# mjuvela/SOC

Hardware: AMD Instinct MI355X
Metric: photon packets/sec (higher is better)
Workload: dtype f32

## Files before the change

### soc_amd/csrc/soc_brick.hip

```cpp
#include "soc_walk.h"
#include "soc_ltree.h"

#include <cstdio>
#include <algorithm>
#include <chrono>
#include <cstdlib>
#include <cstring>
#include <vector>

#include "soc_lbricks.h"

#define SOC_BRICK_T 256

#if defined(SOC_BRICK_PROF)
__device__ unsigned long long g_soc_prof[24];
#define SOC_PROF_DECL unsigned int prof_[8] = { 0, 0, 0, 0, 0, 0, 0, 0 }, dprof_[8] = { 0, 0, 0, 0, 0, 0, 0, 0 };  unsigned long long tprof_[8] = { 0, 0, 0, 0, 0, 0, 0, 0 }, tlast_ = __builtin_readcyclecounter()
#define SOC_PROF_T(i) do { const unsigned long long t_ = __builtin_readcyclecounter();  tprof_[i] += t_ - tlast_;  tlast_ = t_; } while (0)
#define SOC_PROF_ENTRY const unsigned long long tentry_ = __builtin_readcyclecounter()
#define SOC_PROF_SINCE_ENTRY(i) do { tprof_[i] += tlast_ - tentry_; } while (0)
#define SOC_PROF(i, n) do { prof_[i] += (unsigned int)(n); } while (0)
#define SOC_DPROF(i, n) do { dprof_[i] += (unsigned int)(n); } while (0)
#define SOC_PROF_FLUSH do { if ((threadIdx.x & 63) == 0) for (int i_ = 0; i_ < 8; i_++) atomicAdd(&g_soc_prof[16 + i_], (unsigned long long)dprof_[i_]); \
                            if ((threadIdx.x & 63) == 0) for (int i_ = 0; i_ < 8; i_++) atomicAdd(&g_soc_prof[i_], (unsigned long long)prof_[i_]); \
                            if ((threadIdx.x & 63) == 0) for (int i_ = 0; i_ < 8; i_++) atomicAdd(&g_soc_prof[8 + i_], tprof_[i_]); } while (0)
extern "C" __attribute__((visibility("default"))) void soc_prof_read(unsigned long long *out, int reset)
{
    (void)hipMemcpyFromSymbol(out, HIP_SYMBOL(g_soc_prof), sizeof(unsigned long long) * 24);
    if (reset) { unsigned long long z[24] = { 0 };  (void)hipMemcpyToSymbol(HIP_SYMBOL(g_soc_prof), z, sizeof(z)); }
}
#else
#define SOC_PROF_DECL
#define SOC_PROF_ENTRY
#define SOC_PROF_SINCE_ENTRY(i) do { } while (0)
#define SOC_PROF_T(i) do { } while (0)
#define SOC_PROF(i, n) do { } while (0)
#define SOC_DPROF(i, n) do { } while (0)
#define SOC_PROF_FLUSH do { } while (0)
#endif
#define SOC_BRICK_PMAX 4096
#define SOC_RANK_BITS 16
#define SOC_LBRICK_PMAX 32768

enum { SOC_BM_STEP = 0, SOC_BM_CLIMB = 1, SOC_BM_SWAP = 3, SOC_BM_IDLE = 4 };

struct __align__(16) SocPk2 { float4 A, B, C; uint4 D; };

struct SocDesc { int brick, start, count, pad; };

#if defined(SOC_BRICK_NT)
#define SOC_NT_LOAD(p)      __builtin_nontemporal_load(p)
#define SOC_NT_STORE(v, p)  __builtin_nontemporal_store((v), (p))
#else
#define SOC_NT_LOAD(p)      (*(p))
#define SOC_NT_STORE(v, p)  (*(p) = (v))
#endif
typedef float soc_f4v __attribute__((ext_vector_type(4)));
typedef uint32_t soc_u2v __attribute__((ext_vector_type(2)));
#define SOC_GLOBAL __attribute__((address_space(1)))
#define SOC_CHUNK_AT(base, slot) ((decltype(base))((SOC_GLOBAL const char *)(base) + (uint32_t)((uint32_t)(slot) << 2)))
#define SOC_TAKE(dst, src) asm volatile("v_mov_b32 %0, %1" : "=v"(dst) : "v"(src))
__device__ __forceinline__ float4 soc_ld4(const float4 *p) { const soc_f4v v = SOC_NT_LOAD((const soc_f4v *)p);  return make_float4(v.x, v.y, v.z, v.w); }
__device__ __forceinline__ void soc_st4(float4 *p, float4 a) { soc_f4v v = { a.x, a.y, a.z, a.w };  SOC_NT_STORE(v, (soc_f4v *)p); }

struct SocBrickArgs {
    int LB, NBX, NBY, NBZ, NB;
    int NBQ;
    int T, P, KCAP, FTH;
    int CTH;
    int TAIL;
    int PARK;
    SocPk2 *pk;
    const uint32_t *idq;
    uint32_t *idq_next;
    uint32_t *keyq;
    uint32_t *posq;
    int *hist;
    int *off;
    const SocDesc *desc;
    const int *ndesc;
    SocDesc *desc_next;
    int *ndesc_next;
    int *total;
    int ev_brick;
    int HS;
    long long opt_stride;
    int target, nl;
    const uint32_t *first;
    int *admit;
    int CAP;
    const float2 *DS;
    float sib_thr;
    const int *bcell;
    const int *bbase;
    int LT;
    int EQ;
    int slow_every;
    const SocLBrick *lbr;
    const float *btree;
    const int *rbrick;
    int kexp;
    int int_only;
    int ali;
    int roi_on;
    SocPk2 *park;
    SocSca sca;
    const float2 *kopt;
    long long kopt_stride;
};

#include "soc_octbricks.h"
#define SOC_LVL_SHIFT 16
#define SOC_LCH_SHIFT 20

__device__ __forceinline__ void soc_qh_init(int *sH, int HS, int NQ)
{
    if (HS == 0) { for (int i = threadIdx.x; i < NQ; i += blockDim.x) sH[i] = 0; }
    else         { for (int i = threadIdx.x; i < HS; i += blockDim.x) { sH[i] = -1;  sH[HS + i] = 0; } }
}
__device__ __forceinline__ int soc_qh_find(int *sH, int HS, int key)
{
    uint32_t h = (((uint32_t)key * 0x9E3779B1u) >> 12) & (uint32_t)(HS - 1);
    for (int t = 0; t < 32; t++) {
        const int old = atomicCAS(&sH[h], -1, key);
        if (old == -1 || old == key) return (int)h;
        h = (h + 1) & (uint32_t)(HS - 1);
    }
    return -1;
}
#define SOC_POS_FINAL 0x80000000u
__device__ __forceinline__ uint32_t soc_qh_rank(int *sH, int HS, int key, int *ghist)
{
    if (HS == 0) return ((uint32_t)key << SOC_RANK_BITS) | (uint32_t)atomicAdd(&sH[key], 1);
    const int h = soc_qh_find(sH, HS, key);
    if (h >= 0) return ((uint32_t)h << SOC_RANK_BITS) | (uint32_t)atomicAdd(&sH[HS + h], 1);
    return SOC_POS_FINAL | (uint32_t)atomicAdd(&ghist[key], 1);
}
__device__ __forceinline__ void soc_qh_bases(int *sH, int HS, int NQ, int *ghist)
{
    if (HS == 0) {
        for (int i = threadIdx.x; i < NQ; i += blockDim.x) { const int c = sH[i];  if (c) sH[i] = atomicAdd(&ghist[i], c); }
    } else {
        for (int i = threadIdx.x; i < HS; i += blockDim.x) { const int k = sH[i], c = sH[HS + i];  if (k >= 0 && c) sH[HS + i] = atomicAdd(&ghist[k], c); }
    }
}
__device__ __forceinline__ uint32_t soc_qh_place(const int *sH, int HS, uint32_t pack)
{
    if (pack & SOC_POS_FINAL) return pack & ~SOC_POS_FINAL;
    return (uint32_t)sH[(HS ? HS : 0) + (pack >> SOC_RANK_BITS)] + (pack & ((1u << SOC_RANK_BITS) - 1u));
}


__device__ __forceinline__ void soc_cell_brick(const SocBrickArgs &A, float px, float py, float pz, int &brick, int &lid)
{
    const int ix = (int)soc_floorf(px), iy = (int)soc_floorf(py), iz = (int)soc_floorf(pz);
    const int M = (1 << A.LB) - 1;
    brick = ((iz >> A.LB) * A.NBY + (iy >> A.LB)) * A.NBX + (ix >> A.LB);
    lid   = ((iz & M) << (2 * A.LB)) | ((iy & M) << A.LB) | (ix & M);
}

struct SocBrickLane {
    float px, py, pz, ux, uy, uz;
    float photons, free_path, tau, dens;
    int   level, ind, scat;
    soc_rng_t rng;

    __device__ __forceinline__ void begin_conditioned(const SocSim &S)
    {
        scat = 0;
        tau  = 0.0f;
        free_path = soc_draw_free_path(S, &rng, photons);
    }
    __device__ __forceinline__ void begin(const SocSim &S)
    {
        if (soc_fabsf(ux) < SOC_DEPS) ux = SOC_DEPS;
        if (soc_fabsf(uy) < SOC_DEPS) uy = SOC_DEPS;
        if (soc_fabsf(uz) < SOC_DEPS) uz = SOC_DEPS;
        soc_normalize(ux, uy, uz);
        scat = 0;
        tau  = 0.0f;
        free_path = soc_draw_free_path(S, &rng, photons);
    }
};


__global__ void soc_brick2_init(const SocSimPack *Kp, SocBrickArgs A, uint32_t count, uint32_t *idq0, SocDesc *desc0, int *ndesc0, int *hist)
{
    const SocSimPack &K = *Kp;
    const uint32_t t = blockIdx.x * blockDim.x + threadIdx.x;
    SocPk2 *pk = A.pk;
    if (t < count) {
        int l = 0, hi = K.n;
        while (hi - l > 1) { const int m = (l + hi) >> 1;  if (t >= K.first[m]) l = m; else hi = m; }
        const soc_rng_t r = soc_seed_stream(K.S[l].seed_mul, K.S[l].seed_tab, K.S[l].gid0 + (t - K.first[l]));
        SocPk2 p;
        p.A = make_float4(0.0f, 0.0f, 0.0f, 0.0f);
        p.B = p.A;
        p.C = make_float4(0.0f, 0.0f, __int_as_float(l << SOC_LCH_SHIFT), __int_as_float(-1));
        const uint32_t cell0 = (K.S[l].SOURCE == SOC_SOURCE_CL) ? (uint32_t)((int)(K.S[l].gid0 + (t - K.first[l])) - K.S[l].GLOBAL) : 0u;
        p.D = make_uint4(r.x, r.c, 0u, cell0);
        pk[t] = p;
        idq0[t] = t;
        if (A.park) { p.C = p.A;  p.D = make_uint4(0u, 0u, 0u, 0u);  A.park[t] = p; }
    }
    const uint32_t active = min(count, (uint32_t)A.target);
    uint32_t dbase = 0;
    for (int l = 0; l < K.n; l++) {
        const uint32_t hi = min(K.first[l + 1], active);
        const uint32_t cnt = (hi > K.first[l]) ? (hi - K.first[l]) : 0u;
        const uint32_t nd = (cnt + A.P - 1) / A.P;
        if (t >= dbase && t < dbase + nd) {
            const uint32_t k = t - dbase;
            SocDesc d;
            d.brick = A.NBQ + A.EQ * l;
// ... 176 lines not shown
                    }
                }
            }
            SOC_PROF_T(2);
            if (finish) {
                if (!CL && (level == level0) && (ind == ind0)) {
                    px += SOC_PEPS * ux;  py += SOC_PEPS * uy;  pz += SOC_PEPS * uz;
                }
                nvisit++;
                if (ind < 0) {
                    mode = SOC_BM_SWAP;  key = A.NBQ + A.EQ * (lsh >> SOC_LCH_SHIFT);
                } else {
                    const int nb = (int)(sl >> SOC_SLOT_BITS);
                    lid = (int)(sl & SOC_SLOT_MASK);
                    if (nb != mybrick || nvisit >= A.KCAP) { mode = SOC_BM_SWAP;  key = qbase + nb; }
                }
            }
        } else
        if (mode == SOC_BM_STEP) {
            const int   oind = ind, lid0 = lid;
            const float p0x = px, p0y = py, p0z = pz, d0 = dens;
            if (ABU) { float2 o = S.OPT[(lsh >> SOC_LCH_SHIFT) * A.opt_stride + oind];  kabs = o.x;  ksca = o.y; }
            float fx, fy, fz;
            if (__ballot(__builtin_fminf(px, __builtin_fminf(py, pz)) < 0.0f) == 0ull) {
                fx = __builtin_amdgcn_fractf(px);  fy = __builtin_amdgcn_fractf(py);  fz = __builtin_amdgcn_fractf(pz);
            } else {
                fx = soc_fmod1f(px);  fy = soc_fmod1f(py);  fz = soc_fmod1f(pz);
            }
            const float ax = soc_div_by_rcp(((ux > 0.0f) ? (1.0f + SOC_PEPS) : -SOC_PEPS) - fx, ux, rux);
            const float ay = soc_div_by_rcp(((uy > 0.0f) ? (1.0f + SOC_PEPS) : -SOC_PEPS) - fy, uy, ruy);
            const float az = soc_div_by_rcp(((uz > 0.0f) ? (1.0f + SOC_PEPS) : -SOC_PEPS) - fz, uz, ruz);
            float ds = __builtin_fminf(ax, __builtin_fminf(ay, az));
            px += ds * ux;
            py += ds * uy;
            pz += ds * uz;
            ds = soc_scale_down(ds, 0);
            const bool inside = (px > 0.0f) & (px < fNX) & (py > 0.0f) & (py < fNY) & (pz > 0.0f) & (pz < fNZ);
            const int ix = inside ? (int)px : 0;
            const int iy = inside ? (int)py : 0;
            const int iz = inside ? (int)pz : 0;
            const int nind = iz * NX * NY + iy * NX + ix;
            const int nb   = ((iz >> LB) * A.NBY + (iy >> LB)) * A.NBX + (ix >> LB);
            const int nlid = ((iz & M) << (2 * LB)) | ((iy & M) << LB) | (ix & M);
            const bool stay = inside & (nb == mybrick);
            const float ndens = G.DENS[nind];
            const float tauA = ds * d0 * kabs;
            const float dtau = ds * d0 * ksca;
            if (free_path < (tau + dtau)) {
                px = p0x;  py = p0y;  pz = p0z;
                mode = SOC_BM_SWAP;  key = A.NBQ + A.EQ * (lsh >> SOC_LCH_SHIFT) + 1;
            } else {
                const float e = (__ballot(!(tauA < 0.34f)) == 0ull) ? soc_expf_small(-tauA) : soc_expf(-tauA);
                const float delta = (tauA > SOC_TAULIM) ? (photons * (1.0f - e)) : (photons * tauA * (1.0f - 0.5f * tauA));
                atomicAdd(&sT[lid0], delta * tw);
                if (WINT) atomicAdd(&sI[lid0], delta);
                n_tally++;
                photons *= e;
                tau += dtau;
                ind = inside ? nind : -1;
                dens = ndens;
                lid = nlid;
                const bool failed = !CL && (ind == oind);
                px += failed ? (SOC_PEPS * ux) : 0.0f;
                py += failed ? (SOC_PEPS * uy) : 0.0f;
                pz += failed ? (SOC_PEPS * uz) : 0.0f;
                nvisit++;
                if (!inside)                          { mode = SOC_BM_SWAP;  key = A.NBQ + A.EQ * (lsh >> SOC_LCH_SHIFT); }
                else if (!stay || nvisit >= A.KCAP)   { mode = SOC_BM_SWAP;  key = qbase + nb; }
            }
        }
    }

    SOC_PROF_FLUSH;
    atomicAdd(&sCtl[1], (int)n_tally);
    __syncthreads();
    if (OCT) {
        const int *cells = A.bcell + A.bbase[mybrick];
        for (int i = threadIdx.x; i < nslot; i += nthr) {
            const float v = sT[i];
            const float vi = WINT ? sI[i] : 0.0f;
            if (v != 0.0f || vi != 0.0f) {
                const int cell = cells[i];
                soc_tally(S.TABS, cell, v);
                if (WINT) soc_tally(K.S[K.gfirst[qbase / A.NB]].INT, cell, vi);
            }
        }
    } else {
        const int B = 1 << A.LB;
        const int bx = mybrick % A.NBX, by = (mybrick / A.NBX) % A.NBY, bz = mybrick / (A.NBX * A.NBY);
        for (int i = threadIdx.x; i < BV; i += nthr) {
            const float v = sT[i];
            const float vi = WINT ? sI[i] : 0.0f;
            if (v != 0.0f || vi != 0.0f) {
                const int ix = bx * B + (i & M), iy = by * B + ((i >> A.LB) & M), iz = bz * B + (i >> (2 * A.LB));
                const int cell = iz * NX * NY + iy * NX + ix;
                soc_tally(S.TABS, cell, v);
                if (WINT) soc_tally(K.S[K.gfirst[qbase / A.NB]].INT, cell, vi);
            }
        }
    }
    soc_qh_bases(sH, A.HS, NQ, A.hist);
    __syncthreads();
    for (int j = threadIdx.x; j < D.count; j += nthr) A.posq[D.start + j] = soc_qh_place(sH, A.HS, sPos[j]);
    if (threadIdx.x == 0 && S.stats) atomicAdd(S.stats + 0, (unsigned long long)(unsigned int)sCtl[1]);
}

#define SOC_LT_ARRIVE 0x80000000u
#define SOC_LQ_SHIFT 24
enum { SOC_OC_STAY = 0, SOC_OC_OWN = 1, SOC_OC_LEAVE = 2, SOC_OC_EXIT = 3, SOC_OC_SLOW = 4, SOC_OC_LOST = 5, SOC_OC_SCAT = 6, SOC_OC_ROI = 7, SOC_OC_DONE = 8,
       SOC_OC_NONE = 9, SOC_OC_IDLE = 10 };
#define SOC_OC_EVQ 0x31020000u
#define SOC_OC_EVQ_OF(oc) ((SOC_OC_EVQ >> ((4 * (oc)) & 31)) & 15u)
static_assert(SOC_OC_EVQ_OF(SOC_OC_EXIT) == 0 && SOC_OC_EVQ_OF(SOC_OC_DONE) == 0 && SOC_OC_EVQ_OF(SOC_OC_SCAT) == 1 && SOC_OC_EVQ_OF(SOC_OC_SLOW) == 2
              && SOC_OC_EVQ_OF(SOC_OC_ROI) == 3 && SOC_OC_DONE == 8 && SOC_OC_NONE == 9, "the event queue of every code that is stored, the wrap of DONE included");
static_assert(SOC_OC_LEAVE == SOC_LT_LEAVE + 1 && SOC_OC_EXIT == SOC_LT_EXIT + 1 && SOC_OC_SLOW == SOC_LT_SLOW + 1 && SOC_OC_LOST == SOC_LT_LOST + 1, "outcome codes follow soc_ltree.h");

__device__ __forceinline__ void soc_cell_coords(const SocGrid &G, const int *sOFF, int level, int ind, int &cx, int &cy, int &cz)
{
    int x = 0, y = 0, z = 0;
    for (int j = 0; j < level; j++) {
        x |= (ind & 1) << j;  y |= ((ind >> 1) & 1) << j;  z |= ((ind >> 2) & 1) << j;
        ind = G.PAR[sOFF[level - j] + ind - G.NXYZ];
    }
    cx = x | ((ind % G.NX) << level);
    cy = y | (((ind / G.NX) % G.NY) << level);
    cz = z | ((ind / (G.NX * G.NY)) << level);
}

__device__ __forceinline__ int soc_cell_index(const SocGrid &G, int level, int cx, int cy, int cz, float &dens)
{
    int ind = ((cz >> level) * G.NY + (cy >> level)) * G.NX + (cx >> level);
    dens = G.DENS[ind];
    for (int l = 1; l <= level; l++) {
        const int sh = level - l;
        ind = soc_link_index(dens) + (((cx >> sh) & 1) | (((cy >> sh) & 1) << 1) | (((cz >> sh) & 1) << 2));
        dens = G.DENS[G.OFF[l] + ind];
    }
    return ind;
}

template <int WINT, bool ALI>
__device__ __forceinline__ void soc_lbrick_tally(float *sT, float *sI, float *sV, float *sX, const int *sC, const int BV, const int st,
                                                 const float delta, const float tw, const float ux, const float uy, const float uz, const uint32_t dw)
{
    if (ALI) atomicAdd((sC[st] == (int)dw) ? &sX[st] : &sT[st], delta * tw);
    else if (WINT != 3) atomicAdd(&sT[st], delta * tw);
    if (WINT) atomicAdd(&sI[st], delta);
    if (WINT == 2) { atomicAdd(&sV[st], delta * ux);  atomicAdd(&sV[BV + st], delta * uy);  atomicAdd(&sV[2 * BV + st], delta * uz); }
}

template <int WINT, bool RAY = false, bool ALI = false, bool LIM = false, bool CART = false, bool ABU = false, bool FLT = false>
__device__ __forceinline__ void soc_lbrick_walk(const SocGrid &G, const SocSimPack &K, const SocBrickArgs &A, const int bid)
{
    if (bid >= *A.ndesc) return;
    SocDesc D = A.desc[bid];
    D.brick = __builtin_amdgcn_readfirstlane(D.brick);  D.start = __builtin_amdgcn_readfirstlane(D.start);  D.count = __builtin_amdgcn_readfirstlane(D.count);
    if (D.brick >= A.NBQ) return;
    const bool parked = __builtin_amdgcn_readfirstlane(D.pad) != 0;
    SOC_PROF_ENTRY;
    const int BV = A.CAP;
    const int nthr = (int)blockDim.x;
    SOC_GLOBAL SocPk2 *pk = (SOC_GLOBAL SocPk2 *)A.pk;

    extern __shared__ float lds[];
    float *sT   = lds;
    float *sI   = sT + ((RAY || WINT == 3) ? 0 : BV);
    float *sV   = sI + (WINT ? BV : 0);
    float *sX   = sV + ((WINT == 2) ? 3 * BV : 0);
    int   *sC   = (int *)(sX + (ALI ? BV : 0));
    float *sD   = (float *)(sC + (ALI ? BV : 0));
    const int NQ = A.NBQ + A.EQ * A.nl + 1;
    const float2 *sK = (const float2 *)(sD + BV);
    int   *sH   = (int *)(sD + BV + (ABU ? 2 * BV : 0));
    int   *sCtl = sH + (A.HS ? 2 * A.HS : ((NQ + 3) & ~3));
    float *sL   = (float *)(sCtl + 4);
    const SocSim &S = K.S[0];
    for (int l = threadIdx.x; l < K.n; l += nthr) {
        sL[4 * l] = K.S[l].ABS;  sL[4 * l + 1] = K.S[l].SCA;  sL[4 * l + 2] = K.S[l].TW;
        sL[4 * l + 3] = __int_as_float(((K.S[l].SOURCE == SOC_SOURCE_CL) ? 1 : 0) | ((LIM && K.S[l].SCAKIND == SOC_SCA_PB + 1) ? 2 : 0));
    }
    const int mybrick = (A.NBQ > A.NB) ? (D.brick % A.NB) : D.brick;
    const int qbase = D.brick - mybrick;
    SocLBrick KB = A.lbr[mybrick];
    KB.x0 = __builtin_amdgcn_readfirstlane(KB.x0);  KB.y0 = __builtin_amdgcn_readfirstlane(KB.y0);  KB.z0 = __builtin_amdgcn_readfirstlane(KB.z0);
    KB.bx = __builtin_amdgcn_readfirstlane(KB.bx);  KB.by = __builtin_amdgcn_readfirstlane(KB.by);  KB.bz = __builtin_amdgcn_readfirstlane(KB.bz);
    KB.base = __builtin_amdgcn_readfirstlane(KB.base);  KB.nslot = __builtin_amdgcn_readfirstlane(KB.nslot);
    if (!parked) {
        const float *src = A.btree + KB.base;
        for (int i = threadIdx.x; i < KB.nslot; i += nthr) {
            sD[i] = src[i];  if (!RAY && WINT != 3) sT[i] = 0.0f;  if (WINT) sI[i] = 0.0f;
            if (WINT == 2) { sV[i] = 0.0f;  sV[BV + i] = 0.0f;  sV[2 * BV + i] = 0.0f; }
            if (ALI) { sX[i] = 0.0f;  sC[i] = A.bcell[KB.base + i]; }
        }
        if (ABU) {
            const float2 *ksrc = A.kopt + (long long)(qbase / A.NB) * A.kopt_stride + KB.base;
            float2 *dst = (float2 *)(sD + BV);
            for (int i = threadIdx.x; i < KB.nslot; i += nthr) dst[i] = ksrc[i];
        }
    }
    soc_qh_init(sH, A.HS, NQ);
    if (threadIdx.x < 2) sCtl[threadIdx.x] = 0;
    if (parked) for (int j = threadIdx.x; j < D.count; j += nthr) A.keyq[D.start + j] = (uint32_t)D.brick;
    __syncthreads();

    int NX = G.NX, NY = G.NY, NZ = G.NZ, Lmax = G.LEVELS - 1, kexp = A.kexp;
    asm volatile("" : "+s"(NX), "+s"(NY), "+s"(NZ), "+s"(Lmax), "+s"(kexp));
    int rx0 = 1, rx1 = 0, ry0 = 1, ry1 = 0, rz0 = 1, rz1 = 0;
    if (!RAY && A.roi_on) {
        const SocRoi *R = S.ROI;
        rx0 = __builtin_amdgcn_readfirstlane(R->ROI[0]);  rx1 = __builtin_amdgcn_readfirstlane(R->ROI[1]);  ry0 = __builtin_amdgcn_readfirstlane(R->ROI[2]);
        ry1 = __builtin_amdgcn_readfirstlane(R->ROI[3]);  rz0 = __builtin_amdgcn_readfirstlane(R->ROI[4]);  rz1 = __builtin_amdgcn_readfirstlane(R->ROI[5]);
    }
    SOC_GLOBAL uint32_t *keyq_c = (SOC_GLOBAL uint32_t *)(A.keyq + D.start);
    const SOC_GLOBAL uint32_t *idq_c = (const SOC_GLOBAL uint32_t *)(A.idq + D.start);
    asm volatile("" : "+s"(pk), "+s"(keyq_c), "+s"(idq_c));
    float px = 0.0f, py = 0.0f, pz = 0.0f, ux = 0.0f, uy = 0.0f, uz = 0.0f;
    float photons = 0.0f, free_path = 0.0f, tau = 0.0f, dens = 0.0f;
    float rux = 1.0f, ruy = 1.0f, ruz = 1.0f;
    float gx = 0.0f, gy = 0.0f, gz = 0.0f;
    float kabs = 0.0f, ksca = 0.0f, tw = 0.0f;
    int   cx = 0, cy = 0, cz = 0, level = 0, slot = 0, obase = 0, nvisit = 0, cslot = 0, lq = 0;
    int   kl = 0;
    int   what = SOC_LTM_STEP;
    bool  nonudge = false;
    bool  dblstep = false;
    uint32_t dz = 0, dw = 0, wid = 0;
    int   oc = SOC_OC_NONE;
    bool  have = false, nhave = false;
    soc_f4v na = { 0.0f, 0.0f, 0.0f, 0.0f }, nb = na, nc = na;
    soc_u2v ndzw = { 0u, 0u };
    uint32_t nwid = 0, nnwid = 0;
    int   nslot = 0, nnslot = 0;
    bool  nnhave = false;
    unsigned int n_tally = 0;
    SOC_PROF_DECL;
    SOC_PROF_SINCE_ENTRY(3);

    while (!parked) {
        {
            SOC_PROF(0, 1);  SOC_PROF(1, __popcll(__ballot(oc == SOC_OC_STAY)));  SOC_PROF(7, __popcll(__ballot(oc == SOC_OC_IDLE)));
            if (D.count < 4 * nthr)  { SOC_DPROF(0, 1);  SOC_DPROF(1, __popcll(__ballot(oc == SOC_OC_IDLE))); }
            if (D.count < 16 * nthr) { SOC_DPROF(2, 1);  SOC_DPROF(3, __popcll(__ballot(oc == SOC_OC_IDLE))); }
            if (__ballot(nhave | nnhave) == 0ull) { SOC_DPROF(4, 1);  SOC_DPROF(5, __popcll(__ballot(oc == SOC_OC_IDLE))); }
            if (A.TAIL > 0 && D.count >= 8 * nthr && __popcll(__ballot(oc == SOC_OC_IDLE)) >= A.TAIL
                && oc == SOC_OC_STAY && what == SOC_LTM_STEP && nvisit > 0) oc = SOC_OC_OWN;
            const unsigned long long m = __ballot(oc - 1u < (unsigned)SOC_OC_NONE);
            const bool nobody_steps = (__ballot(oc == SOC_OC_STAY) == 0ull);
            if (m != 0ull && (nobody_steps || __popcll(m) >= A.FTH)) {
                SOC_PROF(4, 1);  SOC_PROF(5, __popcll(m));
                if (oc - 1u < (unsigned)SOC_OC_NONE) {
                    const int n_res = atomicAdd(&sCtl[0], 1);
                    const int  n_cz = __float_as_int(nc.w);
                    const int  n_lq = (int)(((uint32_t)n_cz >> SOC_LQ_SHIFT) & (SOC_MAXLAUNCH - 1));
                    const bool n_arrive = (ndzw.y & SOC_LT_ARRIVE) != 0u;
                    const int  n_level = (int)(ndzw.x >> 29);
                    const int  n_ix = n_arrive ? (int)soc_floorf(na.x) : __float_as_int(nc.y), n_iy = n_arrive ? (int)soc_floorf(na.y) : __float_as_int(nc.z),
                               n_iz = n_arrive ? (int)soc_floorf(na.z) : (n_cz & ((1 << SOC_LQ_SHIFT) - 1));
                    int n_s2 = SOC_MAD24(SOC_MAD24(n_iz - KB.z0, KB.by, n_iy - KB.y0), KB.bx, n_ix - KB.x0);
                    n_s2 = ((unsigned)n_s2 < (unsigned)KB.nslot) ? n_s2 : 0;
                    const soc_f4v l4 = *(const soc_f4v *)&sL[4 * n_lq];
                    const float n_rec = sD[n_s2];
                    if (have) {
                        SOC_GLOBAL SocPk2 *q = pk + wid;
                        { const soc_f4v v = { px, py, pz, photons };  SOC_NT_STORE(v, (SOC_GLOBAL soc_f4v *)&q->A); }
                        { const soc_f4v v = { tau, __int_as_float(cx), __int_as_float(cy), __int_as_float(cz | (lq << SOC_LQ_SHIFT)) };  SOC_NT_STORE(v, (SOC_GLOBAL soc_f4v *)&q->C); }
                        q->D.z = dz | ((uint32_t)level << 29);
                        q->D.w = dw | (((oc == SOC_OC_LEAVE) | (oc == SOC_OC_SLOW)) ? SOC_LT_ARRIVE : 0u);
                        if (LIM) SOC_NT_STORE(free_path, &q->B.w);
                        const int evk = A.NBQ + A.EQ * lq + (int)SOC_OC_EVQ_OF(oc);
                        const int key = (oc == SOC_OC_OWN) ? D.brick : ((oc == SOC_OC_LEAVE) ? kl : ((oc == SOC_OC_LOST) ? (NQ - 1) : evk));
                        SOC_NT_STORE((uint32_t)key, SOC_CHUNK_AT(keyq_c, cslot));
                    }
                    have = nhave;
                    wid = nwid;  cslot = nslot;
                    SOC_TAKE(px, na.x);  SOC_TAKE(py, na.y);  SOC_TAKE(pz, na.z);  SOC_TAKE(photons, na.w);
                    SOC_TAKE(ux, nb.x);  SOC_TAKE(uy, nb.y);  SOC_TAKE(uz, nb.z);  SOC_TAKE(free_path, nb.w);
                    SOC_TAKE(tau, nc.x);
                    dz = ndzw.x & 0x1fffffffu;  dw = ndzw.y & ~SOC_LT_ARRIVE;
                    level = n_level;
                    lq = n_lq;
                    kabs = l4.x;  ksca = l4.y;  tw = l4.z;  nonudge = RAY || ((__float_as_int(l4.w) & 1) != 0);
                    if (LIM) dblstep = (__float_as_int(l4.w) & 2) != 0;
                    nvisit = 0;
                    oc = have ? SOC_OC_STAY : oc;
                    obase = -1;
                    {
                        const bool settled = CART || ((n_level == 0) && (!n_arrive || ((n_rec > 0.0f) && !(!RAY && A.roi_on))));
                        what = settled ? SOC_LTM_STEP : (n_arrive ? SOC_LTM_ARRIVE : SOC_LTM_PLACE);
                        slot = settled ? n_s2 : -1;  dens = settled ? n_rec : dens;
                        cx = settled ? n_ix : __float_as_int(nc.y);  cy = settled ? n_iy : __float_as_int(nc.z);  cz = settled ? n_iz : (n_cz & ((1 << SOC_LQ_SHIFT) - 1));
                    }
                    nhave = nnhave;
                    nwid = nnwid;  nslot = nnslot;
                    asm volatile("" : "+v"(nwid), "+v"(na), "+v"(nb), "+v"(nc), "+v"(ndzw) : "v"(cx), "v"(cy), "v"(cz), "v"(dz), "v"(dw), "v"(level), "v"(what) : "memory");
                    if (nhave) {
                        const SOC_GLOBAL SocPk2 *q = pk + nwid;
                        na = SOC_NT_LOAD((const SOC_GLOBAL soc_f4v *)&q->A);  nb = SOC_NT_LOAD((const SOC_GLOBAL soc_f4v *)&q->B);  nc = SOC_NT_LOAD((const SOC_GLOBAL soc_f4v *)&q->C);
                        ndzw = *(const SOC_GLOBAL soc_u2v *)&q->D.z;
                    }
                    nnslot = n_res;
                    nnhave = nnslot < D.count;
                    if (nnhave) nnwid = SOC_NT_LOAD(SOC_CHUNK_AT(idq_c, nnslot));
                    rux = 1.0f / ux;  ruy = 1.0f / uy;  ruz = 1.0f / uz;
                    gx = (ux > 0.0f) ? (1.0f + SOC_PEPS) : -SOC_PEPS;  gy = (uy > 0.0f) ? (1.0f + SOC_PEPS) : -SOC_PEPS;  gz = (uz > 0.0f) ? (1.0f + SOC_PEPS) : -SOC_PEPS;
                    if (!have) oc = (nhave | nnhave) ? SOC_OC_NONE : SOC_OC_IDLE;
                }
            }
        }
        SOC_PROF_T(0);
        if (__ballot(oc != SOC_OC_IDLE) == 0ull) break;
#if defined(SOC_BRICK_PROF)
        int prof_trips = 0;
#endif
        if (oc == SOC_OC_STAY) {
            bool move = true;
            const int slot0 = slot;
            float tauA = 0.0f, dtau = 0.0f;
            if (what == SOC_LTM_STEP) {
                if (ABU) { const float2 o = sK[slot];  kabs = o.x;  ksca = o.y; }
                const float p0x = px, p0y = py, p0z = pz;
                float fx, fy, fz;
                if (__ballot(__builtin_fminf(px, __builtin_fminf(py, pz)) < 0.0f) == 0ull) {
                    fx = __builtin_amdgcn_fractf(px);  fy = __builtin_amdgcn_fractf(py);  fz = __builtin_amdgcn_fractf(pz);
                } else {
                    fx = soc_fmod1f(px);  fy = soc_fmod1f(py);  fz = soc_fmod1f(pz);
                }
                const float ax = soc_div_by_rcp(gx - fx, ux, rux);
                const float ay = soc_div_by_rcp(gy - fy, uy, ruy);
                const float az = soc_div_by_rcp(gz - fz, uz, ruz);
                float ds = __builtin_fminf(ax, __builtin_fminf(ay, az));
                px += ds * ux;
                py += ds * uy;
                pz += ds * uz;
                ds = ds * soc_lt_pow2(-level);
                tauA = ds * dens * kabs;
                dtau = ds * dens * (RAY ? photons : ksca);
                bool scat = free_path < (tau + dtau);
                if (LIM) {
                    const bool lim = free_path < 0.0f;
                    float d = (-free_path < ds) ? -free_path : ds;
                    d = dblstep ? (float)((double)d + 1.0e-6) : (d + 1.0e-6f);
                    d = lim ? d : ds;
                    dtau = d * dens * photons;
                    free_path = lim ? (free_path + d) : free_path;
                    const bool stop = lim & !(free_path < 0.0f);
                    scat = !lim & (free_path < (tau + dtau));
                    tau = stop ? (tau + dtau) : tau;
                    n_tally += stop ? 1u : 0u;
                    oc = stop ? SOC_OC_DONE : SOC_OC_STAY;
                    move = !stop;
                }
                px = scat ? p0x : px;  py = scat ? p0y : py;  pz = scat ? p0z : pz;
                oc = scat ? SOC_OC_SCAT : oc;
                move = move & !scat;
            }
            if (CART) {
                if (move) {
                    n_tally++;
                    tau += dtau;
                    const int  ix = (int)soc_floorf(px), iy = (int)soc_floorf(py), iz = (int)soc_floorf(pz);
                    const bool outside = (px == 0.0f) | (py == 0.0f) | (pz == 0.0f)
                                         | ((unsigned)ix >= (unsigned)NX) | ((unsigned)iy >= (unsigned)NY) | ((unsigned)iz >= (unsigned)NZ);
                    const int  rx = ix - KB.x0, ry = iy - KB.y0, rz = iz - KB.z0;
                    const bool inbox = !(((unsigned)rx >= (unsigned)KB.bx) | ((unsigned)ry >= (unsigned)KB.by) | ((unsigned)rz >= (unsigned)KB.bz));
                    const bool inside = inbox & !outside;
                    const int  ns = inside ? SOC_MAD24(SOC_MAD24(rz, KB.by, ry), KB.bx, rx) : slot0;
                    const float rec = sD[ns];
                    const float nz = (inside & !nonudge & (ns == slot0)) ? SOC_PEPS : 0.0f;
                    px += nz * ux;  py += nz * uy;  pz += nz * uz;
                    slot = ns;  dens = rec;
                    cx = inside ? ix : cx;  cy = inside ? iy : cy;  cz = inside ? iz : cz;
                    nvisit += inside ? 1 : 0;
                    kl = -1 - SOC_MAD24(SOC_MAD24(iz, NY, iy), NX, ix);
                    oc = inside ? ((nvisit >= A.KCAP) ? SOC_OC_OWN : SOC_OC_STAY) : (outside ? SOC_OC_EXIT : SOC_OC_LEAVE);
                }
                SOC_PROF_T(2);
            } else
            if (move) {
                SocLtAim AM;
                if (FLT) soc_lt_aim_flt(KB, NX, NY, NZ, Lmax, what, px, py, pz, level, cx, cy, cz, obase, AM);
                else     soc_lt_aim(KB, NX, NY, NZ, Lmax, kexp, what, px, py, pz, level, cx, cy, cz, obase, AM);
                int   r = AM.r;
                const float rec = sD[AM.s];
                if ((A.slow_every > 0) && (what == SOC_LTM_STEP) && (level > 0) && (((n_tally + 1u + wid) % (unsigned)A.slow_every) == 0u)) r = SOC_LT_SLOW;
                float delta = 0.0f;
                int   st = 0;
                {
                    const bool stepped = (what == SOC_LTM_STEP);
                    n_tally += stepped ? 1u : 0u;
                    tau += dtau;
                    if (!RAY) {
                        const float e = (__ballot(!(tauA < 0.34f)) == 0ull) ? soc_expf_small(-tauA) : soc_expf(-tauA);
                        delta = (tauA > SOC_TAULIM) ? (photons * (1.0f - e)) : (photons * tauA * (1.0f - 0.5f * tauA));
                        st = stepped ? slot0 : 0;
                        photons *= e;
                    }
                }
                SOC_PROF_T(1);
                const int orx = cx >> level, ory = cy >> level, orz = cz >> level;
#if defined(SOC_BRICK_PROF)
                const bool prof_lands = (r == SOC_LT_INSIDE);
#endif
                if (FLT) { if (r == SOC_LT_INSIDE) r = soc_lt_land_flt(sD, AM, Lmax, what, rec, px, py, pz, level, cx, cy, cz, slot, obase, dens); }
                else if (r == SOC_LT_INSIDE) r = soc_lt_land(sD, AM, Lmax, what, rec, px, py, pz, level, cx, cy, cz, slot, obase, dens);
#if defined(SOC_BRICK_PROF)
                prof_trips = prof_lands ? (level - AM.l) : 0;
#endif
                if (!RAY) soc_lbrick_tally<WINT, ALI>(sT, sI, sV, sX, sC, BV, st, delta, tw, ux, uy, uz, dw);
                const bool inside = (r == SOC_LT_INSIDE);
                const bool moved  = inside & (what != SOC_LTM_PLACE);
                const float nz = (moved & !nonudge & (slot == slot0)) ? SOC_PEPS : 0.0f;
                px += nz * ux;  py += nz * uy;  pz += nz * uz;
                nvisit += moved ? 1 : 0;
                kl = -1 - SOC_MAD24(SOC_MAD24(AM.Rz, NY, AM.Ry), NX, AM.Rx);
                oc = inside ? ((moved & (nvisit >= A.KCAP)) ? SOC_OC_OWN : SOC_OC_STAY) : (r + 1);
                if (!RAY && A.roi_on) {
                    const int nrx = cx >> level, nry = cy >> level, nrz = cz >> level;
                    const bool was = (orx >= rx0) & (orx <= rx1) & (ory >= ry0) & (ory <= ry1) & (orz >= rz0) & (orz <= rz1);
                    const bool is  = (nrx >= rx0) & (nrx <= rx1) & (nry >= ry0) & (nry <= ry1) & (nrz >= rz0) & (nrz <= rz1);
                    const bool entered = moved & is & !was;
                    oc = entered ? SOC_OC_ROI : oc;
                }
                what = SOC_LTM_STEP;
            }
            SOC_PROF_T(2);
        }
#if defined(SOC_BRICK_PROF)
        {
            int wtrips = 0;
            for (int t = 1; t < SOC_MAXL; t++) wtrips += (__ballot(prof_trips >= t) != 0ull) ? 1 : 0;
            SOC_PROF(2, wtrips);  SOC_PROF(3, __popcll(__ballot(prof_trips >= 1)));  SOC_PROF(6, (wtrips >= 2) ? 1 : 0);
        }
#endif
    }

    SOC_PROF_T(5);
    atomicAdd(&sCtl[1], (int)n_tally);
    __syncthreads();
    SOC_PROF_T(6);
    if (!parked && !RAY) {
        const int *cells = A.bcell + KB.base;
        for (int i = threadIdx.x; i < KB.nslot; i += nthr) {
            const float vi = WINT ? sI[i] : 0.0f;
            const float v = (WINT == 3) ? (vi * K.S[K.gfirst[qbase / A.NB]].TW) : sT[i];
            if (v != 0.0f || vi != 0.0f || (ALI && sX[i] != 0.0f)) {
                const int cell = cells[i];
                soc_tally(S.TABS, cell, v);
                if (WINT) soc_tally(K.S[K.gfirst[qbase / A.NB]].INT, cell, vi);
                if (ALI && (sX[i] != 0.0f)) soc_tally(S.XAB, cell, sX[i]);
                if (WINT == 2) {
                    float *IV = K.S[K.gfirst[qbase / A.NB]].INTV;
                    const long C = K.S[0].CELLS;
                    soc_tally(IV, cell, sV[i]);  soc_tally(IV + C, cell, sV[BV + i]);  soc_tally(IV + 2 * C, cell, sV[2 * BV + i]);
                }
            }
        }
    }
    SOC_PROF_T(7);
    for (int j = threadIdx.x; j < D.count; j += nthr) {
        int k = (int)A.keyq[D.start + j];
        if (k < 0) { k = qbase + A.rbrick[-1 - k];  A.keyq[D.start + j] = (uint32_t)k; }
        A.posq[D.start + j] = soc_qh_rank(sH, A.HS, k, A.hist);
    }
    __syncthreads();
    soc_qh_bases(sH, A.HS, NQ, A.hist);
    __syncthreads();
    for (int j = threadIdx.x; j < D.count; j += nthr) A.posq[D.start + j] = soc_qh_place(sH, A.HS, A.posq[D.start + j]);
    if (!RAY && threadIdx.x == 0 && S.stats) atomicAdd(S.stats + 0, (unsigned long long)(unsigned int)sCtl[1]);
    if (RAY && threadIdx.x == 0 && S.stats) atomicAdd(S.stats + 3, (unsigned long long)(unsigned int)sCtl[1]);
    SOC_PROF_T(4);
    SOC_PROF_FLUSH;
}


template <bool OCT, typename W>
__device__ __forceinline__ bool soc_roi_create(const SocGrid &G, const SocSim &S, const int *sOFF, const int id, int &III, W &w)
{
    const SocRoi &R = *S.ROI;
    const int relem = id % R.NELEM;
    int   iside = relem, rside;
    float RDX, RDY;
    const float rd = (float)G.NX / ((float)R.DIM[0]);
    if (iside < (R.DIM[1] * R.DIM[2])) {
        RDX = ((float)(iside % R.DIM[1]) + 0.5f) * rd;  RDY = ((float)(iside / R.DIM[1]) + 0.5f) * rd;  rside = 0;
    } else {
        iside -= R.DIM[1] * R.DIM[2];
        if (iside < (R.DIM[0] * R.DIM[2])) {
            RDX = ((float)(iside % R.DIM[0]) + 0.5f) * rd;  RDY = ((float)(iside / R.DIM[0]) + 0.5f) * rd;  rside = 1;
        } else {
            iside -= R.DIM[0] * R.DIM[2];
            rside = 3;
            RDX = 0.0f;  RDY = 0.0f;
            if (iside < (R.DIM[0] * R.DIM[1])) {
                RDX = ((float)(iside % R.DIM[0]) + 0.5f) * rd;  RDY = ((float)(iside / R.DIM[0]) + 0.5f) * rd;  rside = 2;
            }
        }
    }
    const float RX0 = (float)((double)(R.NSIDE * R.NSIDE) * 12.0 / (100.0 * (double)S.BATCH));
    const int npix = 12 * R.NSIDE * R.NSIDE;
    while (III < S.BATCH) {
        const int pix = III % npix;
        III++;
        w.photons = RX0 * R.LOAD[(size_t)relem * npix + pix];
        if (w.photons <= 0.0f) continue;
        float v1, v2, s1, c1, s2, c2;
        soc_pixel2angles_ring(R.NSIDE, pix, v1, v2);
        v1 += (soc_rand(&w.rng) - 0.5f) * 0.05f;
        v2 += (soc_rand(&w.rng) - 0.5f) * 0.05f;
        soc_sincosf(v1, &s1, &c1);
        soc_sincosf(v2, &s2, &c2);
        w.ux = s2 * c1;  w.uy = s2 * s1;  w.uz = c2;
        if (rside == 0) {
            w.py = RDX + (-0.49f + 0.98f * soc_rand(&w.rng)) * rd;  w.pz = RDY + (-0.49f + 0.98f * soc_rand(&w.rng)) * rd;
            w.px = (w.ux > 0.0f) ? SOC_PEPS : ((float)G.NX - SOC_PEPS);
        }
        if (rside == 1) {
            w.px = RDX + (-0.49f + 0.98f * soc_rand(&w.rng)) * rd;  w.pz = RDY + (-0.49f + 0.98f * soc_rand(&w.rng)) * rd;
            w.py = (w.uy > 0.0f) ? SOC_PEPS : ((float)G.NY - SOC_PEPS);
        }
        if (rside == 2) {
            w.px = RDX + (-0.49f + 0.98f * soc_rand(&w.rng)) * rd;  w.py = RDY + (-0.49f + 0.98f * soc_rand(&w.rng)) * rd;
            w.pz = (w.uz > 0.0f) ? SOC_PEPS : ((float)G.NZ - SOC_PEPS);
        }
        soc_indexg<OCT>(G, sOFF, w.px, w.py, w.pz, w.level, w.ind, w.dens);
        return true;
    }
    return false;
}

template <bool OCT, bool ABU, int WINT, int KIND, bool LT, bool FLT = false>
__device__ __forceinline__ void soc_brick_events(const SocGrid &G, const SocSimPack &K, const SocBrickArgs &A, const int ebid, const int slice)
{
    constexpr int  SRC = (KIND == 3) ? 1 : -1;
    const int di = A.ndesc[2] + ebid;
    if (di >= *A.ndesc) return;
    SocDesc D = A.desc[di];
    if (D.brick < A.NBQ) return;
    {
        const int first = (int)(slice * blockDim.x);
        if (first >= D.count) return;
        D.start += first;
        D.count = min((int)blockDim.x, D.count - first);
    }
    SocPk2 *pk = A.pk;
    const int NQ = A.NBQ + A.EQ * K.n + 1;
    const int lq = (D.brick - A.NBQ) / A.EQ;
    const SocSim &S = K.S[lq];
    const int  skind = (KIND == 4) ? ((S.SOURCE == SOC_SOURCE_CL) ? 2 : (S.SOURCE == SOC_SOURCE_HP) ? 1 : 0) : KIND;
    const bool CL = (skind == 2), HP = (skind == 1);
    const int qbase = (A.NBQ > A.NB) ? K.grp[lq] * A.NB : 0;
    extern __shared__ float lds[];
    int   *sH   = (int *)lds;
    int   *sCtl = sH + (A.HS ? 2 * A.HS : NQ);
    int   *sOFF = sCtl + 4;
    soc_qh_init(sH, A.HS, NQ);
    if (threadIdx.x < 4) sCtl[threadIdx.x] = 0;
    if (threadIdx.x < SOC_MAXL) sOFF[threadIdx.x] = G.OFF[threadIdx.x];
    __syncthreads();
    unsigned int n_tally = 0, n_pkt = 0, n_scat = 0;
    uint32_t mypack = 0;

    for (int j = threadIdx.x; j < D.count; j += blockDim.x) {
        const uint32_t wid = A.idq[D.start + j];
        SocPk2 p = pk[wid];
        SocBrickLane w;
        w.px = p.A.x;  w.py = p.A.y;  w.pz = p.A.z;  w.photons = p.A.w;
        w.ux = p.B.x;  w.uy = p.B.y;  w.uz = p.B.z;  w.free_path = p.B.w;
        w.tau = p.C.x;  w.dens = p.C.y;
        int lid = __float_as_int(p.C.z) & 0xffff;
        w.level = OCT ? ((__float_as_int(p.C.z) >> SOC_LVL_SHIFT) & 15) : 0;
        w.ind = __float_as_int(p.C.w);
        w.rng.x = p.D.x;  w.rng.c = p.D.y;
        int III = (int)(p.D.z & 0xffffffu);
        w.scat = (int)(p.D.z >> 24);
        int key = (int)p.D.w;
        uint32_t cl_cell = p.D.w;
        const int evk = (D.brick - A.NBQ) % A.EQ;
        bool create = (evk == 0);
        int ccx = 0, ccy = 0, ccz = 0;
        if (LT) {
            ccx = __float_as_int(p.C.y);  ccy = __float_as_int(p.C.z);  ccz = __float_as_int(p.C.w) & ((1 << SOC_LQ_SHIFT) - 1);
            w.level = (int)(p.D.z >> 29);
            w.scat  = (int)((p.D.z >> 24) & 31u);
            if (evk == 2) cl_cell = p.D.w & ~SOC_LT_ARRIVE;
            w.ind = -1;
            if (!create) w.ind = soc_cell_index(G, w.level, ccx, ccy, ccz, w.dens);
        }
        bool mirrored = false;
        if (LT && create && (S.MIRROR > 0)) {
            const bool started = CL ? (((int)cl_cell >= 0) && (III > 0)) : (III > 0);
            if (started) {
                if (FLT) {
                    soc_lt_rootpos_f(w.px, w.py, w.pz, w.level, ccx, ccy, ccz);
                } else if (w.level > 0) {
                    const float sc = soc_lt_pow2(-w.level);
                    w.px = SOC_FMA(w.px, sc, (float)(ccx & ~1) * sc);  w.py = SOC_FMA(w.py, sc, (float)(ccy & ~1) * sc);  w.pz = SOC_FMA(w.pz, sc, (float)(ccz & ~1) * sc);
                }
                soc_mirror<true>(G, sOFF, S.MIRROR, w.px, w.py, w.pz, w.ux, w.uy, w.uz, w.level, w.ind, w.dens);
                mirrored = (w.ind >= 0);
            }
        }
        if (LT && (evk == 3)) {
            soc_roi_save(G, sOFF, *S.ROI, w.px, w.py, w.pz, w.ux, w.uy, w.uz, w.level, w.ind, w.photons);
            key = qbase + A.rbrick[((ccz >> w.level) * G.NY + (ccy >> w.level)) * G.NX + (ccx >> w.level)];
        } else
        if (LT && (evk == 2)) {
            const int ind0 = w.ind, level0 = w.level;
            if (FLT) soc_index<true, float>(G, sOFF, w.px, w.py, w.pz, w.level, w.ind, w.dens);
// ... 1286 lines not shown
```

Baseline: 490.6 million.

## Batch brick preload and tally flush loads, prefetch cell indices across barrier

Brick loading now issues eight global loads per thread before any LDS store, so misses overlap instead of serialising. The descriptor, brick record and per-sim parameters are loaded word by word up front, and LDS zeroing is split out from the loads. The tally flush prefetches cell indices before the barrier, software-pipelines the next batch of indices, and uses wave-uniform global pointers with relaxed agent-scope atomics. This adds register pressure and a dependence on asm barriers to hold the loads in place.

New measurement: 499.6 million, median of 6. 1.02x the previous value.

```diff
diff --git a/soc_amd/csrc/soc_brick.hip b/soc_amd/csrc/soc_brick.hip
--- a/soc_amd/csrc/soc_brick.hip
+++ b/soc_amd/csrc/soc_brick.hip
@@ -40,12 +40,16 @@
 #define SOC_BRICK_PMAX 4096
 #define SOC_RANK_BITS 16
 #define SOC_LBRICK_PMAX 32768
+#define SOC_LB_BATCH 8
+#define SOC_LANDED8(a) asm volatile("" : "+v"(a[0]), "+v"(a[1]), "+v"(a[2]), "+v"(a[3]), "+v"(a[4]), "+v"(a[5]), "+v"(a[6]), "+v"(a[7]))
+static_assert(SOC_LB_BATCH == 8, "SOC_LANDED8 names the values of a batch one by one");
 
 enum { SOC_BM_STEP = 0, SOC_BM_CLIMB = 1, SOC_BM_SWAP = 3, SOC_BM_IDLE = 4 };
 
 struct __align__(16) SocPk2 { float4 A, B, C; uint4 D; };
 
 struct SocDesc { int brick, start, count, pad; };
+static_assert(sizeof(SocDesc) == 16 && sizeof(SocLBrick) == 32, "soc_lbrick_walk reads both word by word");
 
 #if defined(SOC_BRICK_NT)
 #define SOC_NT_LOAD(p)      __builtin_nontemporal_load(p)
@@ -56,9 +60,24 @@
 #endif
 typedef float soc_f4v __attribute__((ext_vector_type(4)));
 typedef uint32_t soc_u2v __attribute__((ext_vector_type(2)));
+typedef float soc_f2v __attribute__((ext_vector_type(2)));
 #define SOC_GLOBAL __attribute__((address_space(1)))
 #define SOC_CHUNK_AT(base, slot) ((decltype(base))((SOC_GLOBAL const char *)(base) + (uint32_t)((uint32_t)(slot) << 2)))
 #define SOC_TAKE(dst, src) asm volatile("v_mov_b32 %0, %1" : "=v"(dst) : "v"(src))
+template <typename T> __device__ __forceinline__ SOC_GLOBAL T *soc_uniform_ptr(SOC_GLOBAL T *p)
+{
+    const uint64_t a = (uint64_t)p;
+    const uint32_t lo = __builtin_amdgcn_readfirstlane((uint32_t)a), hi = __builtin_amdgcn_readfirstlane((uint32_t)(a >> 32));
+    return (SOC_GLOBAL T *)(((uint64_t)hi << 32) | lo);
+}
+__device__ __forceinline__ void soc_tally_g(SOC_GLOBAL float *buf, int cell, float v)
+{
+#if defined(SOC_EXPERIMENT_NO_TALLY)
+    if (v == 1.2345e-30f) buf[cell] = v;
+#else
+    __hip_atomic_fetch_add(buf + cell, v, __ATOMIC_RELAXED, __HIP_MEMORY_SCOPE_AGENT);
+#endif
+}
 __device__ __forceinline__ float4 soc_ld4(const float4 *p) { const soc_f4v v = SOC_NT_LOAD((const soc_f4v *)p);  return make_float4(v.x, v.y, v.z, v.w); }
 __device__ __forceinline__ void soc_st4(float4 *p, float4 a) { soc_f4v v = { a.x, a.y, a.z, a.w };  SOC_NT_STORE(v, (soc_f4v *)p); }
 
@@ -541,11 +560,16 @@
 template <int WINT, bool RAY = false, bool ALI = false, bool LIM = false, bool CART = false, bool ABU = false, bool FLT = false>
 __device__ __forceinline__ void soc_lbrick_walk(const SocGrid &G, const SocSimPack &K, const SocBrickArgs &A, const int bid)
 {
-    if (bid >= *A.ndesc) return;
-    SocDesc D = A.desc[bid];
+    const SOC_GLOBAL int *descp = (const SOC_GLOBAL int *)(A.desc + bid);
+    const int nd = *(const SOC_GLOBAL int *)A.ndesc;
+    SocDesc D = { descp[0], descp[1], descp[2], descp[3] };
+    int Kn = *(const SOC_GLOBAL int *)&K.n;
+    asm volatile("" : "+v"(D.brick), "+v"(D.start), "+v"(D.count), "+v"(D.pad), "+v"(Kn));
+    if (bid >= nd) return;
     D.brick = __builtin_amdgcn_readfirstlane(D.brick);  D.start = __builtin_amdgcn_readfirstlane(D.start);  D.count = __builtin_amdgcn_readfirstlane(D.count);
     if (D.brick >= A.NBQ) return;
     const bool parked = __builtin_amdgcn_readfirstlane(D.pad) != 0;
+    Kn = __builtin_amdgcn_readfirstlane(Kn);
     SOC_PROF_ENTRY;
     const int BV = A.CAP;
     const int nthr = (int)blockDim.x;
@@ -564,32 +588,64 @@
     int   *sCtl = sH + (A.HS ? 2 * A.HS : ((NQ + 3) & ~3));
     float *sL   = (float *)(sCtl + 4);
     const SocSim &S = K.S[0];
-    for (int l = threadIdx.x; l < K.n; l += nthr) {
+    const int mybrick = (A.NBQ > A.NB) ? (D.brick % A.NB) : D.brick;
+    const int qbase = D.brick - mybrick;
+    const SOC_GLOBAL int *lbrp = (const SOC_GLOBAL int *)(A.lbr + mybrick);
+    SocLBrick KB = { lbrp[0], lbrp[1], lbrp[2], lbrp[3], lbrp[4], lbrp[5], lbrp[6], lbrp[7] };
+    const SOC_GLOBAL SocSim *Sl = (const SOC_GLOBAL SocSim *)K.S + min((int)threadIdx.x, Kn - 1);
+    const float l_abs = Sl->ABS, l_sca = Sl->SCA, l_tw = Sl->TW;
+    const int l_source = Sl->SOURCE, l_scakind = LIM ? Sl->SCAKIND : 0;
+    if (!parked) {
+        for (int i = threadIdx.x; i < BV; i += nthr) {
+            if (!RAY && WINT != 3) sT[i] = 0.0f;
+            if (WINT) sI[i] = 0.0f;
+            if (WINT == 2) { sV[i] = 0.0f;  sV[BV + i] = 0.0f;  sV[2 * BV + i] = 0.0f; }
+            if (ALI) sX[i] = 0.0f;
+        }
+    }
+    soc_qh_init(sH, A.HS, NQ);
+    if (threadIdx.x < 2) sCtl[threadIdx.x] = 0;
+    if (parked) for (int j = threadIdx.x; j < D.count; j += nthr) A.keyq[D.start + j] = (uint32_t)D.brick;
+    if ((int)threadIdx.x < Kn) {
+        const int l = threadIdx.x;
+        sL[4 * l] = l_abs;  sL[4 * l + 1] = l_sca;  sL[4 * l + 2] = l_tw;
+        sL[4 * l + 3] = __int_as_float(((l_source == SOC_SOURCE_CL) ? 1 : 0) | ((LIM && l_scakind == SOC_SCA_PB + 1) ? 2 : 0));
+    }
+    for (int l = threadIdx.x + nthr; l < Kn; l += nthr) {
         sL[4 * l] = K.S[l].ABS;  sL[4 * l + 1] = K.S[l].SCA;  sL[4 * l + 2] = K.S[l].TW;
         sL[4 * l + 3] = __int_as_float(((K.S[l].SOURCE == SOC_SOURCE_CL) ? 1 : 0) | ((LIM && K.S[l].SCAKIND == SOC_SCA_PB + 1) ? 2 : 0));
     }
-    const int mybrick = (A.NBQ > A.NB) ? (D.brick % A.NB) : D.brick;
-    const int qbase = D.brick - mybrick;
-    SocLBrick KB = A.lbr[mybrick];
     KB.x0 = __builtin_amdgcn_readfirstlane(KB.x0);  KB.y0 = __builtin_amdgcn_readfirstlane(KB.y0);  KB.z0 = __builtin_amdgcn_readfirstlane(KB.z0);
     KB.bx = __builtin_amdgcn_readfirstlane(KB.bx);  KB.by = __builtin_amdgcn_readfirstlane(KB.by);  KB.bz = __builtin_amdgcn_readfirstlane(KB.bz);
     KB.base = __builtin_amdgcn_readfirstlane(KB.base);  KB.nslot = __builtin_amdgcn_readfirstlane(KB.nslot);
     if (!parked) {
-        const float *src = A.btree + KB.base;
-        for (int i = threadIdx.x; i < KB.nslot; i += nthr) {
-            sD[i] = src[i];  if (!RAY && WINT != 3) sT[i] = 0.0f;  if (WINT) sI[i] = 0.0f;
-            if (WINT == 2) { sV[i] = 0.0f;  sV[BV + i] = 0.0f;  sV[2 * BV + i] = 0.0f; }
-            if (ALI) { sX[i] = 0.0f;  sC[i] = A.bcell[KB.base + i]; }
-        }
-        if (ABU) {
-            const float2 *ksrc = A.kopt + (long long)(qbase / A.NB) * A.kopt_stride + KB.base;
-            float2 *dst = (float2 *)(sD + BV);
-            for (int i = threadIdx.x; i < KB.nslot; i += nthr) dst[i] = ksrc[i];
-        }
-    }
-    soc_qh_init(sH, A.HS, NQ);
-    if (threadIdx.x < 2) sCtl[threadIdx.x] = 0;
-    if (parked) for (int j = threadIdx.x; j < D.count; j += nthr) A.keyq[D.start + j] = (uint32_t)D.brick;
+        const SOC_GLOBAL float *src = (const SOC_GLOBAL float *)A.btree + KB.base;
+        const SOC_GLOBAL int *csrc = (const SOC_GLOBAL int *)A.bcell + KB.base;
+        const SOC_GLOBAL soc_f2v *ksrc = (const SOC_GLOBAL soc_f2v *)A.kopt + (ABU ? ((long long)(qbase / A.NB) * A.kopt_stride + KB.base) : 0);
+        soc_f2v *dK = (soc_f2v *)(sD + BV);
+        const int last = KB.nslot - 1;
+        for (int i0 = threadIdx.x; i0 < KB.nslot; i0 += SOC_LB_BATCH * nthr) {
+            float d[SOC_LB_BATCH];  int c[SOC_LB_BATCH];  soc_f2v k[SOC_LB_BATCH];
+#pragma unroll
+            for (int u = 0; u < SOC_LB_BATCH; u++) {
+                const int i = min(i0 + u * nthr, last);
+                d[u] = src[i];
+                if (ALI) c[u] = csrc[i];
+                if (ABU) k[u] = ksrc[i];
+            }
+            SOC_LANDED8(d);
+            if (ALI) SOC_LANDED8(c);
+#pragma unroll
+            for (int u = 0; u < SOC_LB_BATCH; u++) {
+                const int i = i0 + u * nthr;
+                if (i <= last) {
+                    sD[i] = d[u];
+                    if (ALI) sC[i] = c[u];
+                    if (ABU) dK[i] = k[u];
+                }
+            }
+        }
+    }
     __syncthreads();
 
     int NX = G.NX, NY = G.NY, NZ = G.NZ, Lmax = G.LEVELS - 1, kexp = A.kexp;
@@ -825,24 +881,63 @@
 
     SOC_PROF_T(5);
     atomicAdd(&sCtl[1], (int)n_tally);
+    const bool flush = !parked && !RAY && KB.nslot > 0;
+    const SOC_GLOBAL int *cells = (const SOC_GLOBAL int *)A.bcell + KB.base;
+    const int last = KB.nslot - 1;
+    SOC_GLOBAL float *gT = nullptr, *gI = nullptr, *gX = nullptr, *gV = nullptr;
+    float gtw = 0.0f;
+    int gcells = 0;
+    int cell[SOC_LB_BATCH];
+    if (flush) {
+        const SOC_GLOBAL SocSim *S0 = (const SOC_GLOBAL SocSim *)K.S;
+        gT = (SOC_GLOBAL float *)S0->TABS;
+        if (ALI) gX = (SOC_GLOBAL float *)S0->XAB;
+        if (WINT == 2) gcells = S0->CELLS;
+        if (WINT) {
+            const SOC_GLOBAL SocSim *Sg = S0 + *((const SOC_GLOBAL int *)K.gfirst + qbase / A.NB);
+            gI = (SOC_GLOBAL float *)Sg->INT;
+            if (WINT == 2) gV = (SOC_GLOBAL float *)Sg->INTV;
+            if (WINT == 3) gtw = Sg->TW;
+        }
+#pragma unroll
+        for (int u = 0; u < SOC_LB_BATCH; u++) cell[u] = cells[min((int)threadIdx.x + u * nthr, last)];
+    }
     __syncthreads();
     SOC_PROF_T(6);
-    if (!parked && !RAY) {
-        const int *cells = A.bcell + KB.base;
-        for (int i = threadIdx.x; i < KB.nslot; i += nthr) {
-            const float vi = WINT ? sI[i] : 0.0f;
-            const float v = (WINT == 3) ? (vi * K.S[K.gfirst[qbase / A.NB]].TW) : sT[i];
-            if (v != 0.0f || vi != 0.0f || (ALI && sX[i] != 0.0f)) {
-                const int cell = cells[i];
-                soc_tally(S.TABS, cell, v);
-                if (WINT) soc_tally(K.S[K.gfirst[qbase / A.NB]].INT, cell, vi);
-                if (ALI && (sX[i] != 0.0f)) soc_tally(S.XAB, cell, sX[i]);
-                if (WINT == 2) {
-                    float *IV = K.S[K.gfirst[qbase / A.NB]].INTV;
-                    const long C = K.S[0].CELLS;
-                    soc_tally(IV, cell, sV[i]);  soc_tally(IV + C, cell, sV[BV + i]);  soc_tally(IV + 2 * C, cell, sV[2 * BV + i]);
-                }
-            }
+    if (flush) {
+        { uint32_t w = __float_as_uint(gtw);  w = __builtin_amdgcn_readfirstlane(w);  gtw = __uint_as_float(w); }
+        gcells = __builtin_amdgcn_readfirstlane(gcells);
+        gT = soc_uniform_ptr(gT);
+        if (WINT) gI = soc_uniform_ptr(gI);
+        if (ALI) gX = soc_uniform_ptr(gX);
+        if (WINT == 2) gV = soc_uniform_ptr(gV);
+        for (int i0 = threadIdx.x; i0 < KB.nslot; i0 += SOC_LB_BATCH * nthr) {
+            float v[SOC_LB_BATCH], vi[SOC_LB_BATCH], vx[SOC_LB_BATCH], v0[SOC_LB_BATCH], v1[SOC_LB_BATCH], v2[SOC_LB_BATCH];
+            int ncell[SOC_LB_BATCH];
+#pragma unroll
+            for (int u = 0; u < SOC_LB_BATCH; u++) {
+                const int i = i0 + u * nthr;
+                const bool in = (i <= last);
+                const int j = in ? i : 0;
+                vi[u] = (WINT && in) ? sI[j] : 0.0f;
+                v[u]  = (WINT == 3) ? (vi[u] * gtw) : (in ? sT[j] : 0.0f);
+                vx[u] = (ALI && in) ? sX[j] : 0.0f;
+                if (WINT == 2) { v0[u] = in ? sV[j] : 0.0f;  v1[u] = in ? sV[BV + j] : 0.0f;  v2[u] = in ? sV[2 * BV + j] : 0.0f; }
+            }
+            const int n0 = i0 + SOC_LB_BATCH * nthr;
+#pragma unroll
+            for (int u = 0; u < SOC_LB_BATCH; u++) ncell[u] = cells[min(n0 + u * nthr, last)];
+#pragma unroll
+            for (int u = 0; u < SOC_LB_BATCH; u++) {
+                if (v[u] != 0.0f || vi[u] != 0.0f || (ALI && vx[u] != 0.0f)) {
+                    soc_tally_g(gT, cell[u], v[u]);
+                    if (WINT) soc_tally_g(gI, cell[u], vi[u]);
+                    if (ALI && (vx[u] != 0.0f)) soc_tally_g(gX, cell[u], vx[u]);
+                    if (WINT == 2) { soc_tally_g(gV, cell[u], v0[u]);  soc_tally_g(gV + (long)gcells, cell[u], v1[u]);  soc_tally_g(gV + 2 * (long)gcells, cell[u], v2[u]); }
+                }
+            }
+#pragma unroll
+            for (int u = 0; u < SOC_LB_BATCH; u++) cell[u] = ncell[u];
         }
     }
     SOC_PROF_T(7);
```
